# Membrizard/ml_conformer_generator

Hardware: AMD Instinct MI355X
Metric: valid molecules/sec @100 diffusion steps (`value` = RAW molecules/s through the whole public path: the reference's validity gate needs RDKit + trained weights, unavailable offline; see `validity`) (higher is better)
Workload: dtype f32

## Files before the change

### include/mlconfgen_hip.h

```cpp
#ifndef MLCONFGEN_HIP_H
#define MLCONFGEN_HIP_H

#include <stdint.h>

#ifdef __cplusplus
extern "C" {
#endif

typedef struct mcg_egnn mcg_egnn;
typedef struct mcg_plan mcg_plan;
typedef struct mcg_gcn mcg_gcn;

const char* mcg_last_error(void);
int mcg_abi_version(void);

int mcg_egnn_create(const float* const* tensors_host, int n_tensors, int hidden, int n_blocks, mcg_egnn** out);
void mcg_egnn_destroy(mcg_egnn* m);
int mcg_egnn_set_precision(mcg_egnn* m, int mode);
enum { MCG_OPT_X6_GEMM = 1, MCG_OPT_GEMM_RN = 2, MCG_OPT_GEMM_X6_RN = 3, MCG_OPT_GEMM_BF16_LDS = 4, MCG_OPT_NODE_FUSED = 5 };
int mcg_egnn_set_option(mcg_egnn* m, int option, int value);

int mcg_debug_gemm_launches(int64_t* counts_host, int reset);

int mcg_plan_create(int B, int N, const int32_t* n_nodes_host, int edge_mt, mcg_plan** out);
typedef struct mcg_plan_opts {
    int32_t edge_mt;
    int32_t n_ranges;
    int32_t four_tile_units;
    int32_t reserved[5];
} mcg_plan_opts;
#define MCG_ALL_FOUR_TILE 0x3fffffff
int mcg_plan_create_ex(int B, int N, const int32_t* n_nodes_host, const mcg_plan_opts* opts, mcg_plan** out);
void mcg_plan_destroy(mcg_plan* p);
int mcg_pool_stats(int64_t* stats_host, int trim);
int mcg_plan_set_latency_mode(mcg_plan* p, int mode);
int mcg_plan_check_tables(int B, int N, const int32_t* n_nodes_host, const mcg_plan_opts* opts, int cus, int32_t* info_host);
int mcg_plan_info(const mcg_plan* p, int32_t* info_host);
int mcg_plan_ranges(const mcg_plan* p);

int mcg_egnn_dynamics(const mcg_egnn* m, mcg_plan* p, const float* t, const float* xh, const float* context,
                      float* out, void* stream);

int mcg_egnn_block_debug(const mcg_egnn* m, mcg_plan* p, int block, float* h_io, float* x_io, const float* x0,
                         void* stream);

int mcg_egnn_gcl_debug(const mcg_egnn* m, mcg_plan* p, int layer, const float* h_in, const float* x_in,
                       const float* x0, void* stream);
int mcg_plan_peek(const mcg_plan* p, int which, float* dst, void* stream);

int mcg_bench_edge(const mcg_egnn* m, mcg_plan* p, int layer, int equiv, int iters, void* stream);
int mcg_bench_edge_incall(const mcg_egnn* m, mcg_plan* p, const float* t, const float* xh, const float* context, float* out,
                          int calls, float* us_host, void* stream);

int mcg_sampler_noise(const mcg_plan* p, const float* randn_x, const float* randn_h, float* eps, void* stream);
int mcg_sampler_step(const mcg_egnn* m, mcg_plan* p, float* z, const float* context, const float* t_dev,
                     const float* randn_x, const float* randn_h, float alpha_ts, float c_eps, float c_noise,
                     float* eps_hat_scratch, void* stream);
int mcg_sampler_decode(const mcg_egnn* m, mcg_plan* p, const float* z0, const float* context, const float* t_zero_dev,
                       const float* randn_x, float inv_alpha0, float sigma0, float sigma_x, float norm_x, float norm_h,
// ... 74 lines not shown
```

### ml_conformer_generator_amd/_lib.py

```python
from __future__ import annotations

import ctypes as C
import os
from typing import Dict, List, Sequence

_HERE = os.path.dirname(os.path.abspath(__file__))
LIB_PATH = os.environ.get("MCG_LIB_PATH") or os.path.join(_HERE, "libmlconfgen_hip.so")

_vp, _i, _f, _d = C.c_void_p, C.c_int, C.c_float, C.c_double
_pp = C.POINTER(C.c_void_p)

SIGNATURES: Dict[str, tuple] = {
    "mcg_last_error": (C.c_char_p, []),
    "mcg_abi_version": (_i, []),
    "mcg_egnn_create": (_i, [_pp, _i, _i, _i, _pp]),
    "mcg_egnn_destroy": (None, [_vp]),
    "mcg_egnn_set_precision": (_i, [_vp, _i]),
    "mcg_egnn_set_option": (_i, [_vp, _i, _i]),
    "mcg_debug_gemm_launches": (_i, [_vp, _i]),
    "mcg_plan_create": (_i, [_i, _i, _vp, _i, _pp]),
    "mcg_plan_create_ex": (_i, [_i, _i, _vp, _vp, _pp]),
    "mcg_plan_destroy": (None, [_vp]),
    "mcg_pool_stats": (_i, [_vp, _i]),
    "mcg_plan_info": (_i, [_vp, _vp]),
    "mcg_plan_ranges": (_i, [_vp]),
    "mcg_plan_set_latency_mode": (_i, [_vp, _i]),
    "mcg_plan_check_tables": (_i, [_i, _i, _vp, _vp, _i, _vp]),
    "mcg_egnn_dynamics": (_i, [_vp, _vp, _vp, _vp, _vp, _vp, _vp]),
    "mcg_egnn_block_debug": (_i, [_vp, _vp, _i, _vp, _vp, _vp, _vp]),
    "mcg_egnn_gcl_debug": (_i, [_vp, _vp, _i, _vp, _vp, _vp, _vp]),
    "mcg_plan_peek": (_i, [_vp, _i, _vp, _vp]),
    "mcg_bench_edge": (_i, [_vp, _vp, _i, _i, _i, _vp]),
    "mcg_bench_edge_incall": (_i, [_vp, _vp, _vp, _vp, _vp, _vp, _i, _vp, _vp]),
    "mcg_sampler_noise": (_i, [_vp, _vp, _vp, _vp, _vp]),
    "mcg_sampler_step": (_i, [_vp, _vp, _vp, _vp, _vp, _vp, _vp, _f, _f, _f, _vp, _vp]),
    "mcg_sampler_decode": (_i, [_vp, _vp, _vp, _vp, _vp, _vp, _f, _f, _f, _f, _f, _vp, _vp, _vp, _vp]),
    "mcg_sampler_blend": (_i, [_vp, _vp, _vp, _vp, _vp, _vp, _f, _f, _f, _i, _vp]),
    "mcg_sampler_noise_keyed": (_i, [_vp, C.c_uint64, _vp, C.c_uint32, C.c_uint32, _vp, _vp, _vp]),
    "mcg_egnn_aggregate": (_i, [_vp, _vp, _vp, _vp, _vp, _i, _i, _vp]),
    "mcg_gcn_create": (_i, [_pp, _i, _pp]),
    "mcg_gcn_destroy": (None, [_vp]),
    "mcg_gcn_forward": (_i, [_vp, _vp, _vp, _vp, _vp, _vp, _i, _vp]),
    "mcg_gcn_check": (_i, [_vp]),
    "mcg_shape_tanimoto": (_i, [_vp, _i, _vp, _vp, _i, _i, _vp, _i, _vp, _i, _f, _f, _vp, _vp, _vp]),
    "mcg_shape_moments": (_i, [_vp, _vp, _i, _i, _d, _d, _f, _i, _i, _vp, _vp, _vp, _vp, _vp]),
    "mcg_shape_frames": (_i, [_vp, _vp, _i, _i, _vp, _vp, _vp, _d, _d, _f, _i, _i, _vp, _vp, _vp]),
    "mcg_shape_frames_tf": (_i, [_vp, _vp, _i, _i, _vp, _vp, _vp, _d, _d, _f, _i, _i, _vp, _vp, _vp, _vp]),
    "mcg_shape_overlay": (_i, [_vp, _i, _vp, _vp, _vp, _vp, _i, _i, _vp, _vp, _i, _f, _f, _vp, _vp, _vp, _vp, _vp, _vp,
                               _vp, _vp]),
    "mcg_shape_overlay_refined": (_i, [_vp, _i, _vp, _vp, _vp, _vp, _i, _i, _vp, _vp, _i, _f, _f, _vp, _vp, _vp, _vp,
                                       _vp, _vp, _vp, _i, _vp, _vp, _vp, _vp, _vp, _vp]),
    "mcg_shape_pair_tanimoto": (_i, [_vp, _vp, _i, _i, _vp, _vp, _i, _f, _f, _vp, _vp, _vp, _vp]),
    "mcg_receptor_overlap": (_i, [_vp, _vp, _vp, _i, _i, _vp, _vp, _i, _i, _vp, _vp, _vp]),
    "mcg_handoff": (_i, [_vp, _vp, _vp, _i, _i, _d, _vp, _vp, _vp, _vp]),
    "mcg_handoff_ex": (_i, [_vp, _vp, _vp, _i, _i, _d, _vp, _vp, _vp, _vp, _vp, _vp, _vp, _vp]),
    "mcg_handoff_elements": (_i, [_vp, _vp, _vp, _i, _i, _d, _vp, _vp, _vp, _vp, _vp, _vp, _vp, _vp, _vp]),
    "mcg_bond_writeback": (_i, [_vp, _vp, _vp, _i, _vp, _vp, _vp]),
    "mcg_ifm_merge": (_i, [_vp, _vp, _i, _vp, _vp, _i, _vp, _vp, _i, _i, _vp, _vp, _vp]),
}



class PlanOpts(C.Structure):
    _fields_ = [("edge_mt", C.c_int32), ("n_ranges", C.c_int32), ("four_tile_units", C.c_int32), ("reserved", C.c_int32 * 5)]


ALL_FOUR_TILE = 0x3fffffff
OPT_X6_GEMM, OPT_GEMM_RN, OPT_GEMM_X6_RN, OPT_GEMM_BF16_LDS, OPT_NODE_FUSED = 1, 2, 3, 4, 5

_lib = None


class McgError(RuntimeError):
    pass


def lib():
    global _lib
    if _lib is not None:
        return _lib
    if not os.path.exists(LIB_PATH):
        raise McgError(
            f"{LIB_PATH} not found: build it with `python -c 'import __graft_entry__ as g; g.build()'` "
            "or `make -C ml_conformer_generator_amd/csrc`. There is no CPU fallback for the hot path.")
    import torch
    handle = C.CDLL(LIB_PATH, mode=C.RTLD_GLOBAL)
    for name, (res, args) in SIGNATURES.items():
        try:
            fn = getattr(handle, name)
        except AttributeError as e:
# ... 32 lines not shown
```

### ml_conformer_generator_amd/csrc/mcg_egnn_api.hip

```cpp
#include "mcg_gemm.h"
#include "mcg_egnn_internal.h"

#include <atomic>
#include <cstring>
#include <utility>

namespace {

constexpr int H = MCG_H, HP = MCG_HP, NT = MCG_NT, IN_NF = MCG_IN_NF;
constexpr float NORM = MCG_NORM;

__global__ __launch_bounds__(128) void k_prep_embed(const float* __restrict__ xh, const float* __restrict__ t,
                                                     const float* __restrict__ ctx, const int* __restrict__ node_mol,
                                                     const int* __restrict__ node_off, int N,
                                                     const float* __restrict__ emb_wT,
                                                     const float* __restrict__ emb_b,
                                                     float* __restrict__ h, float* __restrict__ x, float* __restrict__ x0) {
    const int v = blockIdx.x;
    const int b = node_mol[v];
    const int i = v - node_off[b];
    const float* src = xh + ((size_t)b * N + i) * 11;
    float f[IN_NF];
#pragma unroll
    for (int k = 0; k < 8; ++k) f[k] = src[3 + k];
// ... 248 lines not shown
}

int run_pab(const mcg_egnn* m, mcg_plan* pl, const Route& r, const EdgeLayer& E, hipStream_t s) {
    if (pl->pab_ready || r.pab.family == GemmFamily::X6) {
        if (int e = apply_pending_x(pl, s)) return e;
    }
    if (pl->pab_ready) { pl->pab_ready = false; return MCG_OK; }
    McgGemmArgs g{};
    g.A1 = pl->h; g.lda1 = HP; g.K1 = H; g.bias = E.pab_bias; g.C = pl->pab; g.ldc = 2 * HP;
    g.M = pl->M; g.n_tiles = 2 * NT; g.n_store = 2 * HP; g.act = MCG_ACT_NONE; g.c_blocked = r.pab_blocked ? 1 : 0;
    if (pl->x_pending) {
        g.side_u = pl->pending_u; g.side_slots = pl->pending_slots; g.side_x = pl->x; g.side_M = pl->M;
        pl->x_pending = false;
    }
    return launch_gemm(m, r.pab, g, E.pab_Bp, E.pab_Bp16, E.pab_Bp16x3, s);
}

int run_gcl(const mcg_egnn* m, mcg_plan* pl, int layer, hipStream_t s, bool keep_agg = false) {
    const Route r = route(m, pl, keep_agg);
    const EdgeLayer& E = m->gcl_edge[layer];
    const NodeLayer& Nl = m->gcl_node[layer];
    const int M = pl->M;
    if (int e = run_pab(m, pl, r, E, s)) return e;
    if (int e = run_edge(pl, r, E, false, pl->P, s)) return e;
    if (r.fused) {
        const EdgeLayer& Nx = (layer & 1) ? m->equiv[layer >> 1] : m->gcl_edge[layer + 1];
        McgNodeFusedArgs a{};
        a.h = pl->h; a.ldh = HP; a.P = pl->P; a.ldp = HP; a.a2_rows = pl->pslots4; a.a2_nsum = pl->pspan;
        a.w3 = Nl.w3_Bp16; a.b3 = Nl.b3; a.w4 = Nl.w4_Bp16; a.b4 = Nl.b4; a.h_out = pl->h2; a.ldo = HP;
        a.wab = Nx.pab_Bp16; a.bab = Nx.pab_bias; a.pab = pl->pab; a.ldpab = 2 * HP; a.pab_blocked = r.pab_blocked ? 1 : 0; a.M = M;
        MCG_HIP(mcg_node_fused_launch(a, s));
        pl->pab_ready = true;
        std::swap(pl->h, pl->h2);
        return MCG_OK;
    }
    McgGemmArgs g{};
    g.A1 = pl->h; g.lda1 = HP; g.K1 = H; g.A2 = pl->agg; g.lda2 = HP; g.K2 = H; g.bias = Nl.b3;
    g.C = pl->t1; g.ldc = HP; g.M = M; g.n_tiles = NT; g.n_store = HP; g.act = MCG_ACT_SILU;
    switch (r.agg) {
        case AggSource::GatherU: g.A2 = pl->U; g.a2_rows = pl->units().node_slots; g.a2_nsum = pl->units().max_span; break;
        case AggSource::GatherP: g.A2 = pl->P; g.a2_rows = pl->pslots4; g.a2_nsum = pl->pspan; break;
        case AggSource::GatherAgg2:
            hipLaunchKernelGGL(k_gather_agg2, dim3(M), dim3(128), 0, s, pl->U, pl->units().node_slots, pl->agg);
            MCG_HIP(hipGetLastError());
            break;
        case AggSource::Combine:
            hipLaunchKernelGGL(k_combine_agg_t, dim3(M), dim3(128), 0, s, pl->P, pl->node_slots, pl->agg);
// ... 31 lines not shown
    return run_equiv(m, pl, block, s);
}

}

extern "C" {

static int dynamics_launch(const mcg_egnn* m, mcg_plan* pl, const float* t, const float* xh, const float* context,
                           float* out, hipStream_t s) {
    if (!pl->subs.empty()) {
        MCG_HIP(hipEventRecord(pl->ev_fork, s));
        for (size_t k = 0; k < pl->subs.size(); ++k) {
            const size_t b0 = (size_t)pl->sub_b0[k];
            MCG_HIP(hipStreamWaitEvent(pl->streams[k], pl->ev_fork, 0));
            if (int e = dynamics_launch(m, pl->subs[k], t + b0, xh + b0 * pl->N * 11, context + b0 * pl->N * 3,
                                        out + b0 * pl->N * 11, pl->streams[k])) return e;
            MCG_HIP(hipEventRecord(pl->ev_join[k], pl->streams[k]));
            MCG_HIP(hipStreamWaitEvent(s, pl->ev_join[k], 0));
        }
        return MCG_OK;
    }
    pl->x_pending = false;
    pl->pab_ready = false;
    if (pl->M > 0) {
        hipLaunchKernelGGL(k_prep_embed, dim3(pl->M), dim3(128), 0, s, xh, t, context, pl->node_mol, pl->node_off, pl->N,
                           m->emb_wT, m->emb_b, pl->h, pl->x, pl->x0);
        MCG_HIP(hipGetLastError());
        for (int b = 0; b < m->n_blocks; ++b)
            if (int e = run_block(m, pl, b, s)) return e;
    }
    hipLaunchKernelGGL(k_output, dim3((pl->M + pl->B + 3) / 4), dim3(256), 0, s, pl->h, pl->x, pl->x0, pl->n_nodes, pl->node_off,
                       pl->node_mol, pl->M, pl->B, pl->N, m->out_w, m->out_b, out, pl->x_pending ? pl->pending_u : (const float*)nullptr,
                       pl->x_pending ? pl->pending_slots : (const int4*)nullptr);
    MCG_HIP(hipGetLastError());
    pl->x_pending = false;
    return MCG_OK;
}

static int dynamics_entry(const mcg_egnn* m, mcg_plan* pl, const float* t, const float* xh, const float* context,
                          float* out, void* stream);

int mcg_egnn_dynamics(const mcg_egnn* m, mcg_plan* pl, const float* t, const float* xh, const float* context,
                      float* out, void* stream) {
    if (!m || !pl || !t || !xh || !context || !out) { mcg_set_error("mcg_egnn_dynamics: null argument"); return MCG_ERR_ARG; }
    const int rc = dynamics_entry(m, pl, t, xh, context, out, stream);
    mcg_plan_mark(pl, (hipStream_t)stream);
    return rc;
}

static int dynamics_entry(const mcg_egnn* m, mcg_plan* pl, const float* t, const float* xh, const float* context,
                          float* out, void* stream) {
    hipStream_t s = (hipStream_t)stream;
    static int use_graph = -1;
// ... 156 lines not shown
```

### ml_conformer_generator_amd/csrc/mcg_egnn_internal.h

```cpp
#pragma once
#include "mcg_common.h"
#include "mcg_api_internal.h"
#include "mcg_plan_host.h"

#include <vector>

constexpr int MCG_H = 420;
constexpr int MCG_HP = 432;
constexpr int MCG_PAB_BLOCKED_FLOATS = 2 * 14 * 32;
constexpr int MCG_NT = 27;
constexpr int MCG_KSTEPS = MCG_H / 4;
constexpr int MCG_IN_NF = 12;
constexpr float MCG_NORM = 100.0f;
constexpr int MCG_GROUP_LDS_FLOATS = 28 * 256;

struct EdgeArgs {
    const float* pab;
    const float* x;
    const float* x0;
    const float* wd;
    const float* wd0;
    const float* Bp;
    const float* b2;
    const float* wv;
// ... 61 lines not shown
        int4* node_slots = nullptr;
        int max_span = 2;
    };
    UnitTables ut[2];
    bool have_alt = false;
    const UnitTables& units() const { return ut[(latency_mode == 0 && have_alt) ? 1 : 0]; }
    float *U = nullptr, *Ux = nullptr;
    int4* pslots4 = nullptr;
    int pspan = 0;
    bool x_pending = false;
    bool pab_ready = false;
    const float* pending_u = nullptr;
    const int4* pending_slots = nullptr;
    std::vector<void*> allocs;
    bool is_sub = false;
    int dev = -1;
    hipEvent_t ev_done = nullptr;
    mutable bool ev_pending = false;
    std::vector<mcg_plan*> subs;
    std::vector<int> sub_b0;
    std::vector<hipStream_t> streams;
    std::vector<hipEvent_t> ev_join;
    hipEvent_t ev_fork = nullptr;
    float* t_buf = nullptr;
    hipStream_t cap_stream = nullptr;
    hipGraphExec_t graph_exec = nullptr;
    std::vector<hipGraphExec_t> retired_graphs;
    const void* g_key[5] = {nullptr, nullptr, nullptr, nullptr, nullptr};
    int graph_failed = 0;
    int key_changes = 0;
    float *xh_stage = nullptr, *ctx_stage = nullptr, *out_stage = nullptr;
    int latency_mode = -1;
    struct EdgeTiming { hipEvent_t t0, t1; bool equiv, used; };
    std::vector<EdgeTiming>* edge_timing = nullptr;
    size_t* edge_timing_next = nullptr;
};

inline void mcg_plan_mark(const mcg_plan* pl, hipStream_t s) {
    if (pl && pl->ev_done && hipEventRecord(pl->ev_done, s) == hipSuccess) pl->ev_pending = true;
    else (void)hipGetLastError();
}

struct mcg_plan_mark_guard {
    const mcg_plan* p; hipStream_t s;
    ~mcg_plan_mark_guard() { mcg_plan_mark(p, s); }
};
// ... 9 lines not shown
```

### ml_conformer_generator_amd/csrc/mcg_egnn_plan.hip

```cpp
#include "mcg_egnn_internal.h"

#include <algorithm>
#include <cstring>

namespace { constexpr int HP = MCG_HP; }

void mcg_plan_mark_done(const mcg_plan* p, void* stream) { mcg_plan_mark(p, (hipStream_t)stream); }
int mcg_plan_B(const mcg_plan* p) { return p->B; }
int mcg_plan_N(const mcg_plan* p) { return p->N; }
const int* mcg_plan_n_nodes(const mcg_plan* p) { return p->n_nodes; }

static int plan_create_single(int B, int N, const int32_t* n_nodes_host, const mcg_plan_opts* opts, mcg_plan** out, hipStream_t* ss_io) {
    if (B < 1 || N < 1 || !n_nodes_host || !out) {
        mcg_set_error("mcg_plan_create: bad arguments");
        return MCG_ERR_ARG;
    }
    int dev = 0, cus = 256;
    if (hipGetDevice(&dev) == hipSuccess) (void)hipDeviceGetAttribute(&cus, hipDeviceAttributeMultiprocessorCount, dev);
    (void)hipGetLastError();
    McgPlanHost H;
    if (int e = mcg_plan_build_host(B, N, n_nodes_host, opts, cus, H)) return e;
    if (!*ss_io) MCG_HIP(hipStreamCreateWithFlags(ss_io, hipStreamNonBlocking));
    const hipStream_t ss = *ss_io;
    mcg_plan* p = new mcg_plan();
    p->B = H.B; p->N = H.N; p->M = H.M; p->n_rows = H.n_rows; p->n_mtiles = H.n_mtiles; p->MT = H.MT; p->n_waves = H.n_waves;
    p->n_pslots = H.n_pslots; p->wgc = H.wgc;
    std::vector<int>&nn = H.nn, &node_off = H.node_off, &node_mol = H.node_mol, &wave_poff = H.wave_poff, &ij = H.ij,
                    &node_slots = H.node_slots;
    McgPlanHost::Set (&ht)[2] = H.ht;
    const int n_sets = H.n_sets, best = H.MT, R = 16 * H.MT;
    const bool slots_ok = H.slots_ok, segs_ok = H.segs_ok;
    if (!segs_ok) {
        mcg_set_error("mcg_plan_create: edge_mt = %d puts more than 16 atoms' rows into one %d-row unit (molecules this "
                      "small need edge_mt = 1)", best, R);
        delete p;
        return MCG_ERR_ARG;
    }
    if (!slots_ok) {
        mcg_set_error("mcg_plan_create: a molecule's edge rows span more than 8 tiles per atom (N > 114 is not supported)");
        delete p;
        return MCG_ERR_ARG;
    }
    int max_uslots = 0;
    for (int k = 0; k < n_sets; ++k) max_uslots = std::max(max_uslots, ht[k].n_uslots);
// ... 66 lines not shown

extern "C" {

void mcg_plan_destroy(mcg_plan* p) {
    if (!p) return;
    int prev_dev = -1;
    if (!p->is_sub) {
        if (hipGetDevice(&prev_dev) != hipSuccess) { (void)hipGetLastError(); prev_dev = -1; }
        if (p->dev >= 0 && prev_dev != p->dev && hipSetDevice(p->dev) != hipSuccess) (void)hipGetLastError();
        if (p->ev_done) {
            if (p->ev_pending && hipEventSynchronize(p->ev_done) != hipSuccess) { (void)hipGetLastError(); (void)hipDeviceSynchronize(); }
        } else if (!p->allocs.empty()) {
            (void)hipDeviceSynchronize();
        }
        for (hipStream_t st : p->streams) (void)hipStreamSynchronize(st);
    }
    if (p->graph_exec) (void)hipGraphExecDestroy(p->graph_exec);
    for (hipGraphExec_t ge : p->retired_graphs) (void)hipGraphExecDestroy(ge);
    if (p->cap_stream) (void)hipStreamDestroy(p->cap_stream);
    for (mcg_plan* q : p->subs) mcg_plan_destroy(q);
    for (hipStream_t st : p->streams) (void)hipStreamDestroy(st);
    for (hipEvent_t e : p->ev_join) (void)hipEventDestroy(e);
    if (p->ev_fork) (void)hipEventDestroy(p->ev_fork);
    for (void* q : p->allocs) mcg_dev_free(q);
    if (p->ev_done) (void)hipEventDestroy(p->ev_done);
    const bool restore = !p->is_sub && prev_dev >= 0 && prev_dev != p->dev;
    delete p;
    if (restore && hipSetDevice(prev_dev) != hipSuccess) (void)hipGetLastError();
}

static int plan_finish(mcg_plan* p, int B, int N, const int32_t* n_nodes_host, const mcg_plan_opts* opts);

int mcg_plan_create(int B, int N, const int32_t* n_nodes_host, int edge_mt, mcg_plan** out) {
    mcg_plan_opts o{};
    o.edge_mt = edge_mt;
    return mcg_plan_create_ex(B, N, n_nodes_host, &o, out);
}

int mcg_plan_create_ex(int B, int N, const int32_t* n_nodes_host, const mcg_plan_opts* opts, mcg_plan** out) {
    const int n_ranges = opts ? opts->n_ranges : 0;
    if (n_ranges < 0 || n_ranges > 4) { mcg_set_error("mcg_plan_create_ex: n_ranges must be 0 (auto) .. 4"); return MCG_ERR_ARG; }
    if (opts)
        for (int k = 0; k < 5; ++k)
            if (opts->reserved[k] != 0) { mcg_set_error("mcg_plan_create_ex: mcg_plan_opts.reserved must be zero"); return MCG_ERR_ARG; }
    mcg_plan* p = nullptr;
    hipStream_t cs = nullptr;
    if (int e = plan_create_single(B, N, n_nodes_host, opts, &p, &cs)) { if (cs) (void)hipStreamDestroy(cs); return e; }
    p->cap_stream = cs;
    if (hipGetDevice(&p->dev) != hipSuccess) { (void)hipGetLastError(); p->dev = -1; }
    if (hipEventCreateWithFlags(&p->ev_done, hipEventDisableTiming) != hipSuccess) { (void)hipGetLastError(); p->ev_done = nullptr; }
    if (int e = plan_finish(p, B, N, n_nodes_host, opts)) {
        mcg_plan_destroy(p);
        return e;
    }
    *out = p;
    return MCG_OK;
}

static int plan_finish(mcg_plan* p, int B, int N, const int32_t* n_nodes_host, const mcg_plan_opts* opts) {
    const int n_ranges = opts ? opts->n_ranges : 0;
    if (int e = mcg_dev_alloc((size_t)B * sizeof(float), (void**)&p->t_buf)) return e;
    p->allocs.push_back(p->t_buf);
    constexpr int BF16_TWO_RANGES_FROM_ATOMS = 2 * 32 * 32;
    int parts = 1;
    if (n_ranges > 0) parts = n_ranges;
    else if (p->MT == 1) parts = p->n_mtiles < 3600 ? 1 : p->n_mtiles < 5200 ? 2 : p->n_mtiles < 14000 ? 3 : 4;
    else parts = p->M >= BF16_TWO_RANGES_FROM_ATOMS ? 2 : 1;
    if (parts < 2 || B < 2 * parts || p->n_rows < 4096) return MCG_OK;
    const std::vector<int> cuts = mcg_plan_range_cuts(B, n_nodes_host, parts);
    for (size_t k = 0; k + 1 < cuts.size(); ++k) {
        const int b0 = cuts[k], b1 = cuts[k + 1];
        mcg_plan* sub = nullptr;
        if (int e = plan_create_single(b1 - b0, N, n_nodes_host + b0, opts, &sub, &p->cap_stream)) return e;
        sub->is_sub = true;
        p->subs.push_back(sub);
        p->sub_b0.push_back(b0);
        hipStream_t st; hipEvent_t ev;
        MCG_HIP(hipStreamCreateWithFlags(&st, hipStreamNonBlocking));
        MCG_HIP(hipEventCreateWithFlags(&ev, hipEventDisableTiming));
        p->streams.push_back(st);
        p->ev_join.push_back(ev);
    }
    MCG_HIP(hipEventCreateWithFlags(&p->ev_fork, hipEventDisableTiming));
    return MCG_OK;
}

int mcg_plan_set_latency_mode(mcg_plan* p, int mode) {
    if (!p || mode < -1 || mode > 1) return MCG_ERR_ARG;
    p->latency_mode = mode;
    for (mcg_plan* q : p->subs) q->latency_mode = mode;
    if (p->graph_exec) { (void)hipGraphExecDestroy(p->graph_exec); p->graph_exec = nullptr; }
    return MCG_OK;
}

int mcg_plan_ranges(const mcg_plan* p) { return p ? (p->subs.empty() ? 1 : (int)p->subs.size()) : 0; }

int mcg_plan_info(const mcg_plan* p, int32_t* info ) {
    if (!p || !info) return MCG_ERR_ARG;
    info[0] = p->M; info[1] = p->n_rows; info[2] = p->MT; info[3] = p->n_waves; info[4] = p->n_pslots;
    info[5] = p->B; info[6] = p->N; info[7] = p->n_mtiles;
    return MCG_OK;
}

int mcg_plan_peek(const mcg_plan* pl, int which, float* dst, void* stream) {
// ... 17 lines not shown
```

### ml_conformer_generator_amd/csrc/mcg_plan_host.cpp

```cpp
#include "mcg_plan_host.h"

#include <algorithm>

int mcg_plan_build_host(int B, int N, const int32_t* n_nodes_host, const mcg_plan_opts* opts, int cus, McgPlanHost& H) {
    if (B < 1 || N < 1 || !n_nodes_host) { mcg_set_error("mcg_plan_create: bad arguments"); return MCG_ERR_ARG; }
    const int edge_mt = opts ? opts->edge_mt : 0;
    const int four_tile = opts ? opts->four_tile_units : 0;
    if (edge_mt != 0 && edge_mt != 1 && edge_mt != 4) { mcg_set_error("mcg_plan_create: edge_mt must be 0 (auto), 1 (16-row tiles) or 4 (64-row units)"); return MCG_ERR_ARG; }
    McgPlanHost* const p = &H;
    p->B = B; p->N = N;
    std::vector<int>&nn = H.nn, &node_off = H.node_off, &row_off = H.row_off;
    nn.assign(B, 0); node_off.assign(B + 1, 0); row_off.assign(B + 1, 0);
    for (int b = 0; b < B; ++b) {
        if (n_nodes_host[b] < 0 || n_nodes_host[b] > N) {
            mcg_set_error("mcg_plan_create: n_nodes[%d]=%d outside [0,%d]", b, n_nodes_host[b], N);
            return MCG_ERR_ARG;
        }
        nn[b] = n_nodes_host[b];
        node_off[b + 1] = node_off[b] + nn[b];
        row_off[b + 1] = row_off[b] + nn[b] * (nn[b] > 0 ? nn[b] - 1 : 0);
        if (node_off[b + 1] > 1000000 || row_off[b + 1] > (1 << 30)) {
            mcg_set_error("mcg_plan_create: batch too large for one plan (%d atoms after molecule %d; limit 1e6 atoms, 2^30 edge rows)",
                          node_off[b + 1], b);
            return MCG_ERR_ARG;
        }
    }
    p->M = node_off[B];
// ... 111 lines not shown
                    const int w = unit_of(u);
                    if (w == prev) continue;
                    prev = w;
                    if (cnt == max_span) return false;
                    const int r = std::max(first, 16 * u);
                    node_slots2[4 * (size_t)v + cnt++] = unit_sbase[w] + wave_ws[u] + (ij[2 * (size_t)r + 1] >> 24);
                }
                span = std::max(span, cnt);
            }
        }
        return true;
    };
    McgPlanHost::Set (&ht)[2] = H.ht;
    int& n_sets = H.n_sets;
    n_sets = 0;
    auto keep = [&](int n_full) {
        McgPlanHost::Set& t = ht[n_sets++];
        t.wg_info = wg_info; t.node_slots = node_slots2; t.n_units = n_units; t.n_full = n_full;
        t.n_uslots = unit_sbase[n_units]; t.span = span;
    };
    if (wgc_ok) {
        const int round = 2 * (cus > 0 ? cus : 256);
        const int r = n_wg_all % round;
        int n_full = r * 512 <= 400 * round ? n_wg_all - r : n_wg_all;
        if (four_tile < 0) n_full = 0;
        else if (four_tile > 0) n_full = (int)std::min<long>((((long)four_tile + 7) / 8) * 8, (long)n_wg_all);
        if (n_full < n_wg_all && build_units(n_full, 4)) keep(n_full);
        wgc_ok = build_units(n_wg_all, 2);
        if (wgc_ok) keep(n_wg_all);
        else if (n_sets > 0) wgc_ok = true;
        else if (build_units(0, 4)) { keep(0); wgc_ok = true; }
    }
    p->wgc = wgc_ok;
    return MCG_OK;
}

extern "C" int mcg_plan_check_tables(int B, int N, const int32_t* n_nodes_host, const mcg_plan_opts* opts, int cus, int32_t* info ) {
    if (B < 1 || N < 1 || !n_nodes_host || !info) { mcg_set_error("mcg_plan_check_tables: bad arguments"); return MCG_ERR_ARG; }
    McgPlanHost H;
    if (int e = mcg_plan_build_host(B, N, n_nodes_host, opts, cus, H)) return e;
    const int n_waves = H.n_waves, M = H.M, MT = H.MT;
    const bool wgc = H.wgc;
    for (int k = 0; k < 8; ++k) info[k] = 0;
    info[0] = H.n_sets;
    if (!H.segs_ok || !H.slots_ok) { mcg_set_error("mcg_plan_check_tables: the batch does not fit the requested edge_mt"); return MCG_ERR_ARG; }
    auto fail = [&](const char* what, int a, int b2) { mcg_set_error("mcg_plan_check_tables: %s (%d, %d)", what, a, b2); return MCG_ERR_STATE; };
    for (int b = 0; b < B; ++b) {
        const int n = H.nn[b];
        for (int i = 0; i < n && n > 1; ++i)
            for (int jj = 0; jj < n - 1; ++jj) {
                const size_t r = (size_t)H.row_off[b] + (size_t)i * (n - 1) + jj;
                if (H.ij[2 * r] != H.node_off[b] + i) return fail("row table: wrong i", b, i);
                if ((H.ij[2 * r + 1] & 0xffffff) != H.node_off[b] + jj + (jj >= i ? 1 : 0)) return fail("row table: wrong j", b, i);
            }
    }
    if (!wgc) return MCG_OK;
    if (MT != 1) return fail("workgroup-level tables on a plan that is not 16-row", MT, 0);
    const int n_wg_all = (n_waves + 3) / 4;
    for (int k = 0; k < H.n_sets; ++k) {
        const McgPlanHost::Set& T = H.ht[k];
        const int n_full = T.n_full;
        const int n_tail = n_full < n_wg_all ? n_waves - 4 * n_full : 0;
        if (T.n_units != n_full + n_tail) return fail("unit count", T.n_units, n_full + n_tail);
// ... 29 lines not shown
                    owner[slot] = v;
                    int found = -1;
                    for (int q = 0; q < 4; ++q) if (T.node_slots[4 * (size_t)v + q] == slot) found = q;
                    if (found < 0) return fail("row's slot missing from its atom's list", (int)r, slot);
                    hits[4 * (size_t)v + found] = 1;
                }
                int used = 0;
                for (int q = 0; q < 4; ++q) {
                    const int sl = T.node_slots[4 * (size_t)v + q];
                    if (sl >= 0) { if (!hits[4 * (size_t)v + q]) return fail("atom lists a slot none of its rows writes", v, sl); ++used; }
                    for (int q2 = 0; q2 < q; ++q2) if (sl >= 0 && T.node_slots[4 * (size_t)v + q2] == sl) return fail("atom lists a slot twice", v, sl);
                }
                span_seen = std::max(span_seen, used);
            }
        }
        for (int sl = 0; sl < T.n_uslots; ++sl) if (owner[sl] < 0) return fail("slot that no row writes", sl, k);
        if (span_seen > T.span) return fail("an atom owns more rows of U than the set says", span_seen, T.span);
        if (k == 0) { info[1] = T.n_units; info[2] = T.n_full; info[3] = T.n_uslots; info[4] = T.span; }
        else { info[5] = T.n_units; info[6] = T.n_uslots; info[7] = T.span; }
    }
    return MCG_OK;
}

std::vector<int> mcg_plan_range_cuts(int B, const int32_t* n_nodes_host, int parts) {
    std::vector<int> cuts{0};
    if (B < 1 || !n_nodes_host) return cuts;
    if (parts > B) parts = B;
    if (parts < 1) parts = 1;
    std::vector<long> cum((size_t)B + 1, 0);
    for (int b = 0; b < B; ++b) cum[b + 1] = cum[b] + (long)n_nodes_host[b] * (n_nodes_host[b] > 0 ? n_nodes_host[b] - 1 : 0);
    int b0 = 0;
    for (int k = 0; k < parts; ++k) {
        int b1 = B;
        if (k + 1 < parts) {
            const long target = cum[B] * (k + 1) / parts;
            b1 = b0 + 1;
            while (b1 < B && cum[b1] < target) ++b1;
            const int last = B - (parts - 1 - k);
            if (b1 > last) b1 = last;
        }
        cuts.push_back(b1);
        b0 = b1;
    }
    return cuts;
}
```

### ml_conformer_generator_amd/csrc/mcg_plan_host.h

```cpp
#pragma once
#include <cstdint>
#include <vector>

#include "../../include/mlconfgen_hip.h"
#include "mcg_error.h"

struct McgPlanHost {
    int B = 0, N = 0, M = 0, n_rows = 0, n_mtiles = 0, MT = 1, n_waves = 0, n_pslots = 0;
    bool wgc = false;
    std::vector<int> nn, node_off, row_off, node_mol, wave_poff, ij, node_slots;
    struct Set { std::vector<int> wg_info, node_slots; int n_units = 0, n_full = 0, n_uslots = 0, span = 2; };
    Set ht[2];
    int n_sets = 0;
    bool slots_ok = true, segs_ok = true;
};

int mcg_plan_build_host(int B, int N, const int32_t* n_nodes_host, const mcg_plan_opts* opts, int cus, McgPlanHost& H);

std::vector<int> mcg_plan_range_cuts(int B, const int32_t* n_nodes_host, int parts);
```

### ml_conformer_generator_amd/egnn.py

```python
from __future__ import annotations

import ctypes as C
import weakref
from typing import Dict, Optional

import torch

from . import _lib
from .config import EGNN_HIDDEN, EGNN_N_BLOCKS
from .weights import edm_spec


class BatchPlan:

    def __init__(self, n_nodes: torch.Tensor, max_n_nodes: int, device: torch.device, edge_mt: int = 0,
                 n_ranges: int = 0, four_tile_units: int = 0):
        L = _lib.lib()
        n_host = n_nodes.detach().to("cpu", torch.int32).contiguous().reshape(-1)
        self.B = int(n_host.numel())
        self.N = int(max_n_nodes)
        self.device = torch.device(device)
        self.n_nodes_host = n_host
        self._h = C.c_void_p()
        opts = _lib.PlanOpts(edge_mt=int(edge_mt), n_ranges=int(n_ranges), four_tile_units=int(four_tile_units))
        with torch.cuda.device(self.device):
            _lib.check(L.mcg_plan_create_ex(self.B, self.N, n_host.data_ptr(), C.byref(opts), C.byref(self._h)),
                       "mcg_plan_create_ex")
        info = torch.zeros(8, dtype=torch.int32)
        _lib.check(L.mcg_plan_info(self._h, info.data_ptr()), "mcg_plan_info")
        (self.n_real_nodes, self.n_real_edges, self.edge_mt, self.n_edge_waves, self.n_pslots, _, _,
         self.n_edge_tiles) = [int(v) for v in info]
        self.n_ranges = int(L.mcg_plan_ranges(self._h))

    @property
    def handle(self):
        return self._h

    def set_latency_mode(self, mode: int) -> None:
        _lib.check(_lib.lib().mcg_plan_set_latency_mode(self._h, int(mode)), "mcg_plan_set_latency_mode")

    def node_mask(self) -> torch.Tensor:
        idx = torch.arange(self.N).unsqueeze(0)
        return (idx < self.n_nodes_host.unsqueeze(1)).to(torch.float32).unsqueeze(2).to(self.device)

    def edge_mask(self) -> torch.Tensor:
        em = getattr(self, "_edge_mask", None)
        if em is None:
# ... 63 lines not shown
            dtype, self.compute_dtype = self.compute_dtype, "f32"
            self.set_precision(dtype)

    @property
    def handle(self):
        if not self._h:
            raise _lib.McgError("EGNNDynamics has no weights loaded")
        return self._h

    def set_precision(self, compute_dtype: str = "f32") -> None:
        if compute_dtype not in ("f32", "bf16", "f32x6"):
            raise ValueError("compute_dtype must be 'f32', 'bf16' or 'f32x6'")
        _lib.check(_lib.lib().mcg_egnn_set_precision(self.handle, {"f32": 0, "bf16": 1, "f32x6": 2}[compute_dtype]),
                   "mcg_egnn_set_precision")
        if compute_dtype != self.compute_dtype:
            self._plans.clear()
        self.compute_dtype = compute_dtype

    def set_option(self, option: int, value: int) -> None:
        _lib.check(_lib.lib().mcg_egnn_set_option(self.handle, int(option), int(value)), "mcg_egnn_set_option")
        self._plans.clear()

    def plan(self, n_nodes: torch.Tensor, max_n_nodes: int, edge_mt: int = 0, four_tile_units: int = 0,
             n_ranges: int = 0) -> BatchPlan:
        if edge_mt == 0 and self.compute_dtype in ("bf16", "f32x6") and int(n_nodes.min()) >= 6:
            edge_mt = 4
        if n_ranges == 0 and edge_mt == 4 and self.compute_dtype == "f32x6":
            nn = n_nodes.reshape(-1).to(torch.long)
            n_ranges = 2 if int((nn * (nn - 1)).sum()) >= 1500 * 16 else 1
        key = (int(max_n_nodes), int(edge_mt), int(four_tile_units), int(n_ranges), tuple(int(v) for v in n_nodes.reshape(-1).tolist()))
        p = self._plans.get(key)
        if p is not None:
            self._plans[key] = self._plans.pop(key)
            return p
        while len(self._plans) >= max(1, self.plan_cache_size):
            self._plans.pop(next(iter(self._plans)))
        p = BatchPlan(n_nodes, max_n_nodes, self.device, edge_mt, n_ranges, four_tile_units)
        self._plans[key] = p
        return p

    def sizes_for(self, node_mask: torch.Tensor) -> torch.Tensor:
        tag = getattr(node_mask, "_mcg_mask_tag", None)
        if tag is not None and tag[1] == node_mask._version:
            return tag[2]
        hit = self._node_mask_ok
        if hit is not None and hit[0]() is node_mask and hit[1] == node_mask._version:
            return hit[2]
        sizes = sizes_from_node_mask(node_mask)
        self._node_mask_ok = (weakref.ref(node_mask), node_mask._version, sizes)
        return sizes

    def release_cached_memory(self) -> dict:
        self._plans.clear()
        self._edge_mask_ok = self._node_mask_ok = None
        stats = torch.zeros(4, dtype=torch.int64)
        with torch.cuda.device(self.device):
            _lib.check(_lib.lib().mcg_pool_stats(stats.data_ptr(), 1), "mcg_pool_stats")
        return dict(zip(("in_use_bytes", "cached_bytes", "driver_allocs", "pool_hits"), (int(v) for v in stats)))

    def check_edge_mask(self, plan: BatchPlan, edge_mask, node_mask=None) -> None:
# ... 69 lines not shown
```

Before: 139.7.

## Add tunable range cuts, phase staggering, and full four-tile units in sub-plans

Range splitting moves into a shared chooser that can size the first batch range to one wave round and can stagger sub-plan streams. With staggering on, each range's first edge kernel waits for the previous range's first edge kernel through events. Sub-plans now build with a concurrent flag that keeps every workgroup on four-tile units instead of trimming the partial last round, since they share the GPU with other streams. The new cut and phase options default off, but the concurrent tail rule applies whenever a batch is split into ranges.

Result: no change. 139.8 (median of 6 runs) (+0.1%).

```diff
diff --git a/include/mlconfgen_hip.h b/include/mlconfgen_hip.h
--- a/include/mlconfgen_hip.h
+++ b/include/mlconfgen_hip.h
@@ -27,14 +27,18 @@
     int32_t edge_mt;
     int32_t n_ranges;
     int32_t four_tile_units;
-    int32_t reserved[5];
+    int32_t range_cut;
+    int32_t range_phase;
+    int32_t reserved[3];
 } mcg_plan_opts;
 #define MCG_ALL_FOUR_TILE 0x3fffffff
+#define MCG_RANGE_CUT_ROUND (-1)
 int mcg_plan_create_ex(int B, int N, const int32_t* n_nodes_host, const mcg_plan_opts* opts, mcg_plan** out);
 void mcg_plan_destroy(mcg_plan* p);
 int mcg_pool_stats(int64_t* stats_host, int trim);
 int mcg_plan_set_latency_mode(mcg_plan* p, int mode);
 int mcg_plan_check_tables(int B, int N, const int32_t* n_nodes_host, const mcg_plan_opts* opts, int cus, int32_t* info_host);
+int mcg_plan_check_ranges(int B, int N, const int32_t* n_nodes_host, const mcg_plan_opts* opts, int cus, int32_t* info_host);
 int mcg_plan_info(const mcg_plan* p, int32_t* info_host);
 int mcg_plan_ranges(const mcg_plan* p);
 
diff --git a/ml_conformer_generator_amd/_lib.py b/ml_conformer_generator_amd/_lib.py
--- a/ml_conformer_generator_amd/_lib.py
+++ b/ml_conformer_generator_amd/_lib.py
@@ -26,6 +26,7 @@
     "mcg_plan_ranges": (_i, [_vp]),
     "mcg_plan_set_latency_mode": (_i, [_vp, _i]),
     "mcg_plan_check_tables": (_i, [_i, _i, _vp, _vp, _i, _vp]),
+    "mcg_plan_check_ranges": (_i, [_i, _i, _vp, _vp, _i, _vp]),
     "mcg_egnn_dynamics": (_i, [_vp, _vp, _vp, _vp, _vp, _vp, _vp]),
     "mcg_egnn_block_debug": (_i, [_vp, _vp, _i, _vp, _vp, _vp, _vp]),
     "mcg_egnn_gcl_debug": (_i, [_vp, _vp, _i, _vp, _vp, _vp, _vp]),
@@ -62,10 +63,12 @@
 
 
 class PlanOpts(C.Structure):
-    _fields_ = [("edge_mt", C.c_int32), ("n_ranges", C.c_int32), ("four_tile_units", C.c_int32), ("reserved", C.c_int32 * 5)]
+    _fields_ = [("edge_mt", C.c_int32), ("n_ranges", C.c_int32), ("four_tile_units", C.c_int32), ("range_cut", C.c_int32),
+                ("range_phase", C.c_int32), ("reserved", C.c_int32 * 3)]
 
 
 ALL_FOUR_TILE = 0x3fffffff
+RANGE_CUT_ROUND = -1
 OPT_X6_GEMM, OPT_GEMM_RN, OPT_GEMM_X6_RN, OPT_GEMM_BF16_LDS, OPT_NODE_FUSED = 1, 2, 3, 4, 5
 
 _lib = None
diff --git a/ml_conformer_generator_amd/csrc/mcg_egnn_api.hip b/ml_conformer_generator_amd/csrc/mcg_egnn_api.hip
--- a/ml_conformer_generator_amd/csrc/mcg_egnn_api.hip
+++ b/ml_conformer_generator_amd/csrc/mcg_egnn_api.hip
@@ -294,7 +294,10 @@
     const NodeLayer& Nl = m->gcl_node[layer];
     const int M = pl->M;
     if (int e = run_pab(m, pl, r, E, s)) return e;
+    if (pl->first_edge_pending && pl->wait_first_edge) MCG_HIP(hipStreamWaitEvent(s, pl->wait_first_edge, 0));
     if (int e = run_edge(pl, r, E, false, pl->P, s)) return e;
+    if (pl->first_edge_pending && pl->ev_first_edge) MCG_HIP(hipEventRecord(pl->ev_first_edge, s));
+    pl->first_edge_pending = false;
     if (r.fused) {
         const EdgeLayer& Nx = (layer & 1) ? m->equiv[layer >> 1] : m->gcl_edge[layer + 1];
         McgNodeFusedArgs a{};
@@ -372,6 +375,7 @@
     }
     pl->x_pending = false;
     pl->pab_ready = false;
+    pl->first_edge_pending = true;
     if (pl->M > 0) {
         hipLaunchKernelGGL(k_prep_embed, dim3(pl->M), dim3(128), 0, s, xh, t, context, pl->node_mol, pl->node_off, pl->N,
                            m->emb_wT, m->emb_b, pl->h, pl->x, pl->x0);
@@ -379,6 +383,8 @@
         for (int b = 0; b < m->n_blocks; ++b)
             if (int e = run_block(m, pl, b, s)) return e;
     }
+    if (pl->first_edge_pending && pl->ev_first_edge) MCG_HIP(hipEventRecord(pl->ev_first_edge, s));
+    pl->first_edge_pending = false;
     hipLaunchKernelGGL(k_output, dim3((pl->M + pl->B + 3) / 4), dim3(256), 0, s, pl->h, pl->x, pl->x0, pl->n_nodes, pl->node_off,
                        pl->node_mol, pl->M, pl->B, pl->N, m->out_w, m->out_b, out, pl->x_pending ? pl->pending_u : (const float*)nullptr,
                        pl->x_pending ? pl->pending_slots : (const int4*)nullptr);
diff --git a/ml_conformer_generator_amd/csrc/mcg_egnn_internal.h b/ml_conformer_generator_amd/csrc/mcg_egnn_internal.h
--- a/ml_conformer_generator_amd/csrc/mcg_egnn_internal.h
+++ b/ml_conformer_generator_amd/csrc/mcg_egnn_internal.h
@@ -107,6 +107,8 @@
     std::vector<hipStream_t> streams;
     std::vector<hipEvent_t> ev_join;
     hipEvent_t ev_fork = nullptr;
+    hipEvent_t ev_first_edge = nullptr, wait_first_edge = nullptr;
+    bool first_edge_pending = false;
     float* t_buf = nullptr;
     hipStream_t cap_stream = nullptr;
     hipGraphExec_t graph_exec = nullptr;
diff --git a/ml_conformer_generator_amd/csrc/mcg_egnn_plan.hip b/ml_conformer_generator_amd/csrc/mcg_egnn_plan.hip
--- a/ml_conformer_generator_amd/csrc/mcg_egnn_plan.hip
+++ b/ml_conformer_generator_amd/csrc/mcg_egnn_plan.hip
@@ -10,7 +10,8 @@
 int mcg_plan_N(const mcg_plan* p) { return p->N; }
 const int* mcg_plan_n_nodes(const mcg_plan* p) { return p->n_nodes; }
 
-static int plan_create_single(int B, int N, const int32_t* n_nodes_host, const mcg_plan_opts* opts, mcg_plan** out, hipStream_t* ss_io) {
+static int plan_create_single(int B, int N, const int32_t* n_nodes_host, const mcg_plan_opts* opts, mcg_plan** out, hipStream_t* ss_io,
+                              bool concurrent = false) {
     if (B < 1 || N < 1 || !n_nodes_host || !out) {
         mcg_set_error("mcg_plan_create: bad arguments");
         return MCG_ERR_ARG;
@@ -19,7 +20,7 @@
     if (hipGetDevice(&dev) == hipSuccess) (void)hipDeviceGetAttribute(&cus, hipDeviceAttributeMultiprocessorCount, dev);
     (void)hipGetLastError();
     McgPlanHost H;
-    if (int e = mcg_plan_build_host(B, N, n_nodes_host, opts, cus, H)) return e;
+    if (int e = mcg_plan_build_host(B, N, n_nodes_host, opts, cus, H, concurrent)) return e;
     if (!*ss_io) MCG_HIP(hipStreamCreateWithFlags(ss_io, hipStreamNonBlocking));
     const hipStream_t ss = *ss_io;
     mcg_plan* p = new mcg_plan();
@@ -132,6 +133,7 @@
     for (hipStream_t st : p->streams) (void)hipStreamDestroy(st);
     for (hipEvent_t e : p->ev_join) (void)hipEventDestroy(e);
     if (p->ev_fork) (void)hipEventDestroy(p->ev_fork);
+    if (p->ev_first_edge) (void)hipEventDestroy(p->ev_first_edge);
     for (void* q : p->allocs) mcg_dev_free(q);
     if (p->ev_done) (void)hipEventDestroy(p->ev_done);
     const bool restore = !p->is_sub && prev_dev >= 0 && prev_dev != p->dev;
@@ -151,8 +153,10 @@
     const int n_ranges = opts ? opts->n_ranges : 0;
     if (n_ranges < 0 || n_ranges > 4) { mcg_set_error("mcg_plan_create_ex: n_ranges must be 0 (auto) .. 4"); return MCG_ERR_ARG; }
     if (opts)
-        for (int k = 0; k < 5; ++k)
+        for (int k = 0; k < 3; ++k)
             if (opts->reserved[k] != 0) { mcg_set_error("mcg_plan_create_ex: mcg_plan_opts.reserved must be zero"); return MCG_ERR_ARG; }
+    if (opts && opts->range_cut < MCG_RANGE_CUT_ROUND) { mcg_set_error("mcg_plan_create_ex: range_cut must be 0, MCG_RANGE_CUT_ROUND or > 0"); return MCG_ERR_ARG; }
+    if (opts && opts->range_phase != 0 && opts->range_phase != 1) { mcg_set_error("mcg_plan_create_ex: range_phase must be 0 or 1"); return MCG_ERR_ARG; }
     mcg_plan* p = nullptr;
     hipStream_t cs = nullptr;
     if (int e = plan_create_single(B, N, n_nodes_host, opts, &p, &cs)) { if (cs) (void)hipStreamDestroy(cs); return e; }
@@ -168,20 +172,21 @@
 }
 
 static int plan_finish(mcg_plan* p, int B, int N, const int32_t* n_nodes_host, const mcg_plan_opts* opts) {
-    const int n_ranges = opts ? opts->n_ranges : 0;
     if (int e = mcg_dev_alloc((size_t)B * sizeof(float), (void**)&p->t_buf)) return e;
     p->allocs.push_back(p->t_buf);
-    constexpr int BF16_TWO_RANGES_FROM_ATOMS = 2 * 32 * 32;
-    int parts = 1;
-    if (n_ranges > 0) parts = n_ranges;
-    else if (p->MT == 1) parts = p->n_mtiles < 3600 ? 1 : p->n_mtiles < 5200 ? 2 : p->n_mtiles < 14000 ? 3 : 4;
-    else parts = p->M >= BF16_TWO_RANGES_FROM_ATOMS ? 2 : 1;
-    if (parts < 2 || B < 2 * parts || p->n_rows < 4096) return MCG_OK;
-    const std::vector<int> cuts = mcg_plan_range_cuts(B, n_nodes_host, parts);
+    McgPlanHost G;
+    G.B = B; G.M = p->M; G.n_rows = p->n_rows; G.n_mtiles = p->n_mtiles; G.MT = p->MT;
+    int dev = 0, cus = 256;
+    if (hipGetDevice(&dev) == hipSuccess) (void)hipDeviceGetAttribute(&cus, hipDeviceAttributeMultiprocessorCount, dev);
+    (void)hipGetLastError();
+    McgPlanRanges R;
+    if (int e = mcg_plan_choose_ranges(G, n_nodes_host, opts, cus, R)) return e;
+    const std::vector<int>& cuts = R.cuts;
+    if (cuts.size() < 3) return MCG_OK;
     for (size_t k = 0; k + 1 < cuts.size(); ++k) {
         const int b0 = cuts[k], b1 = cuts[k + 1];
         mcg_plan* sub = nullptr;
-        if (int e = plan_create_single(b1 - b0, N, n_nodes_host + b0, opts, &sub, &p->cap_stream)) return e;
+        if (int e = plan_create_single(b1 - b0, N, n_nodes_host + b0, opts, &sub, &p->cap_stream, true)) return e;
         sub->is_sub = true;
         p->subs.push_back(sub);
         p->sub_b0.push_back(b0);
@@ -190,6 +195,8 @@
         MCG_HIP(hipEventCreateWithFlags(&ev, hipEventDisableTiming));
         p->streams.push_back(st);
         p->ev_join.push_back(ev);
+        if (R.phase && k + 2 < cuts.size()) MCG_HIP(hipEventCreateWithFlags(&sub->ev_first_edge, hipEventDisableTiming));
+        if (R.phase && k > 0) sub->wait_first_edge = p->subs[k - 1]->ev_first_edge;
     }
     MCG_HIP(hipEventCreateWithFlags(&p->ev_fork, hipEventDisableTiming));
     return MCG_OK;
diff --git a/ml_conformer_generator_amd/csrc/mcg_plan_host.cpp b/ml_conformer_generator_amd/csrc/mcg_plan_host.cpp
--- a/ml_conformer_generator_amd/csrc/mcg_plan_host.cpp
+++ b/ml_conformer_generator_amd/csrc/mcg_plan_host.cpp
@@ -2,7 +2,8 @@
 
 #include <algorithm>
 
-int mcg_plan_build_host(int B, int N, const int32_t* n_nodes_host, const mcg_plan_opts* opts, int cus, McgPlanHost& H) {
+int mcg_plan_build_host(int B, int N, const int32_t* n_nodes_host, const mcg_plan_opts* opts, int cus, McgPlanHost& H,
+                        bool concurrent) {
     if (B < 1 || N < 1 || !n_nodes_host) { mcg_set_error("mcg_plan_create: bad arguments"); return MCG_ERR_ARG; }
     const int edge_mt = opts ? opts->edge_mt : 0;
     const int four_tile = opts ? opts->four_tile_units : 0;
@@ -160,7 +161,7 @@
     if (wgc_ok) {
         const int round = 2 * (cus > 0 ? cus : 256);
         const int r = n_wg_all % round;
-        int n_full = r * 512 <= 400 * round ? n_wg_all - r : n_wg_all;
+        int n_full = concurrent || r * 512 > 400 * round ? n_wg_all : n_wg_all - r;
         if (four_tile < 0) n_full = 0;
         else if (four_tile > 0) n_full = (int)std::min<long>((((long)four_tile + 7) / 8) * 8, (long)n_wg_all);
         if (n_full < n_wg_all && build_units(n_full, 4)) keep(n_full);
@@ -173,10 +174,10 @@
     return MCG_OK;
 }
 
-extern "C" int mcg_plan_check_tables(int B, int N, const int32_t* n_nodes_host, const mcg_plan_opts* opts, int cus, int32_t* info ) {
-    if (B < 1 || N < 1 || !n_nodes_host || !info) { mcg_set_error("mcg_plan_check_tables: bad arguments"); return MCG_ERR_ARG; }
+static int check_tables(int B, int N, const int32_t* n_nodes_host, const mcg_plan_opts* opts, int cus, bool concurrent,
+                        int32_t* info ) {
     McgPlanHost H;
-    if (int e = mcg_plan_build_host(B, N, n_nodes_host, opts, cus, H)) return e;
+    if (int e = mcg_plan_build_host(B, N, n_nodes_host, opts, cus, H, concurrent)) return e;
     const int n_waves = H.n_waves, M = H.M, MT = H.MT;
     const bool wgc = H.wgc;
     for (int k = 0; k < 8; ++k) info[k] = 0;
@@ -252,13 +253,50 @@
     return MCG_OK;
 }
 
-std::vector<int> mcg_plan_range_cuts(int B, const int32_t* n_nodes_host, int parts) {
+extern "C" int mcg_plan_check_tables(int B, int N, const int32_t* n_nodes_host, const mcg_plan_opts* opts, int cus, int32_t* info ) {
+    if (B < 1 || N < 1 || !n_nodes_host || !info) { mcg_set_error("mcg_plan_check_tables: bad arguments"); return MCG_ERR_ARG; }
+    return check_tables(B, N, n_nodes_host, opts, cus, false, info);
+}
+
+extern "C" int mcg_plan_check_ranges(int B, int N, const int32_t* n_nodes_host, const mcg_plan_opts* opts, int cus, int32_t* info ) {
+    if (B < 1 || N < 1 || !n_nodes_host || !info) { mcg_set_error("mcg_plan_check_ranges: bad arguments"); return MCG_ERR_ARG; }
+    for (int k = 0; k < 16; ++k) info[k] = 0;
+    McgPlanHost H;
+    if (int e = mcg_plan_build_host(B, N, n_nodes_host, opts, cus, H)) return e;
+    McgPlanRanges R;
+    if (int e = mcg_plan_choose_ranges(H, n_nodes_host, opts, cus, R)) return e;
+    const int parts = (int)R.cuts.size() - 1;
+    if (parts < 1 || parts > 4 || R.cuts.front() != 0 || R.cuts.back() != B) {
+        mcg_set_error("mcg_plan_check_ranges: bad range cuts (%d ranges)", parts);
+        return MCG_ERR_STATE;
+    }
+    info[0] = parts; info[1] = R.phase ? 1 : 0;
+    for (int k = 0; k <= parts; ++k) info[2 + k] = R.cuts[k];
+    for (int k = 0; k < parts; ++k) {
+        const int b0 = R.cuts[k], b1 = R.cuts[k + 1];
+        if (b1 <= b0) { mcg_set_error("mcg_plan_check_ranges: empty range %d", k); return MCG_ERR_STATE; }
+        if (parts == 1) { info[7] = H.wgc ? H.ht[0].n_full : 0; info[11] = H.wgc ? H.ht[0].n_units : 0; break; }
+        int32_t sub[8];
+        if (int e = check_tables(b1 - b0, N, n_nodes_host + b0, opts, cus, true, sub)) return e;
+        info[7 + k] = sub[0] > 0 ? sub[2] : 0;
+        info[11 + k] = sub[0] > 0 ? sub[1] : 0;
+    }
+    return MCG_OK;
+}
+
+std::vector<int> mcg_plan_range_cuts(int B, const int32_t* n_nodes_host, int parts, long first_rows) {
     std::vector<int> cuts{0};
     if (B < 1 || !n_nodes_host) return cuts;
     if (parts > B) parts = B;
     if (parts < 1) parts = 1;
     std::vector<long> cum((size_t)B + 1, 0);
     for (int b = 0; b < B; ++b) cum[b + 1] = cum[b] + (long)n_nodes_host[b] * (n_nodes_host[b] > 0 ? n_nodes_host[b] - 1 : 0);
+    if (first_rows > 0 && parts > 1) {
+        int b1 = 1;
+        while (b1 < B - (parts - 1) && cum[b1 + 1] <= first_rows) ++b1;
+        for (int c : mcg_plan_range_cuts(B - b1, n_nodes_host + b1, parts - 1)) cuts.push_back(b1 + c);
+        return cuts;
+    }
     int b0 = 0;
     for (int k = 0; k < parts; ++k) {
         int b1 = B;
@@ -274,3 +312,24 @@
     }
     return cuts;
 }
+
+int mcg_plan_choose_ranges(const McgPlanHost& H, const int32_t* n_nodes_host, const mcg_plan_opts* opts, int cus, McgPlanRanges& R) {
+    const int n_ranges = opts ? opts->n_ranges : 0, range_cut = opts ? opts->range_cut : 0, range_phase = opts ? opts->range_phase : 0;
+    if (n_ranges < 0 || n_ranges > 4) { mcg_set_error("mcg_plan_create_ex: n_ranges must be 0 (auto) .. 4"); return MCG_ERR_ARG; }
+    if (range_cut < MCG_RANGE_CUT_ROUND) { mcg_set_error("mcg_plan_create_ex: range_cut must be 0, MCG_RANGE_CUT_ROUND or > 0"); return MCG_ERR_ARG; }
+    if (range_phase != 0 && range_phase != 1) { mcg_set_error("mcg_plan_create_ex: range_phase must be 0 or 1"); return MCG_ERR_ARG; }
+    const int B = H.B;
+    R.cuts = {0, B};
+    R.phase = false;
+    constexpr int BF16_TWO_RANGES_FROM_ATOMS = 2 * 32 * 32;
+    int parts = 1;
+    if (n_ranges > 0) parts = n_ranges;
+    else if (H.MT == 1) parts = H.n_mtiles < 3600 ? 1 : H.n_mtiles < 5200 ? 2 : H.n_mtiles < 14000 ? 3 : 4;
+    else parts = H.M >= BF16_TWO_RANGES_FROM_ATOMS ? 2 : 1;
+    if (parts < 2 || B < 2 * parts || H.n_rows < 4096) return MCG_OK;
+    const long round_rows = 2L * (cus > 0 ? cus : 256) * 64;
+    const long first_rows = range_cut == MCG_RANGE_CUT_ROUND ? round_rows : (long)range_cut * 64;
+    R.cuts = mcg_plan_range_cuts(B, n_nodes_host, parts, first_rows);
+    R.phase = range_phase == 1;
+    return MCG_OK;
+}
diff --git a/ml_conformer_generator_amd/csrc/mcg_plan_host.h b/ml_conformer_generator_amd/csrc/mcg_plan_host.h
--- a/ml_conformer_generator_amd/csrc/mcg_plan_host.h
+++ b/ml_conformer_generator_amd/csrc/mcg_plan_host.h
@@ -15,6 +15,10 @@
     bool slots_ok = true, segs_ok = true;
 };
 
-int mcg_plan_build_host(int B, int N, const int32_t* n_nodes_host, const mcg_plan_opts* opts, int cus, McgPlanHost& H);
+int mcg_plan_build_host(int B, int N, const int32_t* n_nodes_host, const mcg_plan_opts* opts, int cus, McgPlanHost& H,
+                        bool concurrent = false);
 
-std::vector<int> mcg_plan_range_cuts(int B, const int32_t* n_nodes_host, int parts);
+std::vector<int> mcg_plan_range_cuts(int B, const int32_t* n_nodes_host, int parts, long first_rows = 0);
+
+struct McgPlanRanges { std::vector<int> cuts; bool phase = false; };
+int mcg_plan_choose_ranges(const McgPlanHost& H, const int32_t* n_nodes_host, const mcg_plan_opts* opts, int cus, McgPlanRanges& R);
diff --git a/ml_conformer_generator_amd/egnn.py b/ml_conformer_generator_amd/egnn.py
--- a/ml_conformer_generator_amd/egnn.py
+++ b/ml_conformer_generator_amd/egnn.py
@@ -14,7 +14,7 @@
 class BatchPlan:
 
     def __init__(self, n_nodes: torch.Tensor, max_n_nodes: int, device: torch.device, edge_mt: int = 0,
-                 n_ranges: int = 0, four_tile_units: int = 0):
+                 n_ranges: int = 0, four_tile_units: int = 0, range_cut: int = 0, range_phase: int = 0):
         L = _lib.lib()
         n_host = n_nodes.detach().to("cpu", torch.int32).contiguous().reshape(-1)
         self.B = int(n_host.numel())
@@ -22,7 +22,8 @@
         self.device = torch.device(device)
         self.n_nodes_host = n_host
         self._h = C.c_void_p()
-        opts = _lib.PlanOpts(edge_mt=int(edge_mt), n_ranges=int(n_ranges), four_tile_units=int(four_tile_units))
+        opts = _lib.PlanOpts(edge_mt=int(edge_mt), n_ranges=int(n_ranges), four_tile_units=int(four_tile_units),
+                             range_cut=int(range_cut), range_phase=int(range_phase))
         with torch.cuda.device(self.device):
             _lib.check(L.mcg_plan_create_ex(self.B, self.N, n_host.data_ptr(), C.byref(opts), C.byref(self._h)),
                        "mcg_plan_create_ex")
@@ -132,20 +133,20 @@
         self._plans.clear()
 
     def plan(self, n_nodes: torch.Tensor, max_n_nodes: int, edge_mt: int = 0, four_tile_units: int = 0,
-             n_ranges: int = 0) -> BatchPlan:
+             n_ranges: int = 0, range_cut: int = 0, range_phase: int = 0) -> BatchPlan:
         if edge_mt == 0 and self.compute_dtype in ("bf16", "f32x6") and int(n_nodes.min()) >= 6:
             edge_mt = 4
         if n_ranges == 0 and edge_mt == 4 and self.compute_dtype == "f32x6":
             nn = n_nodes.reshape(-1).to(torch.long)
             n_ranges = 2 if int((nn * (nn - 1)).sum()) >= 1500 * 16 else 1
-        key = (int(max_n_nodes), int(edge_mt), int(four_tile_units), int(n_ranges), tuple(int(v) for v in n_nodes.reshape(-1).tolist()))
+        key = (int(max_n_nodes), int(edge_mt), int(four_tile_units), int(n_ranges), int(range_cut), int(range_phase), tuple(int(v) for v in n_nodes.reshape(-1).tolist()))
         p = self._plans.get(key)
         if p is not None:
             self._plans[key] = self._plans.pop(key)
             return p
         while len(self._plans) >= max(1, self.plan_cache_size):
             self._plans.pop(next(iter(self._plans)))
-        p = BatchPlan(n_nodes, max_n_nodes, self.device, edge_mt, n_ranges, four_tile_units)
+        p = BatchPlan(n_nodes, max_n_nodes, self.device, edge_mt, n_ranges, four_tile_units, range_cut, range_phase)
         self._plans[key] = p
         return p
 
```
